# broadinstitute/permutect

Measured on AMD Instinct MI355X. Metric: read-sets/sec (train fwd+bwd), higher is better.
Workload: dtype f32 (fp32 accumulate; fwd: 2 x f16 pieces per operand = 23 bits; bwd: 2 x bf16 pieces = 16 bits)

## Files before the change

permutect_amd/csrc/pmt_phi.hip:

```cpp
#include <hip/hip_runtime.h>
#include <math.h>

#include "permutect_amd.h"

#define PHI_THREADS 256
#define PHI_MAXN (2 * PMT_MAX_ORTHO_DIM)
#define PHI_MAX_SQUARINGS 1100

__device__ double block_max(double v, double* red) {
    const int tid = threadIdx.x;
    red[tid] = v;
    __syncthreads();
    for (int s = PHI_THREADS / 2; s > 0; s >>= 1) {
        if (tid < s) red[tid] = fmax(red[tid], red[tid + s]);
        __syncthreads();
    }
    const double r = red[0];
    __syncthreads();
    return r;
}
__device__ double block_sum(double v, double* red) {
    const int tid = threadIdx.x;
    red[tid] = v;
    __syncthreads();
    for (int s = PHI_THREADS / 2; s > 0; s >>= 1) {
        if (tid < s) red[tid] += red[tid + s];
        __syncthreads();
    }
    const double r = red[0];
    __syncthreads();
    return r;
}

__device__ void matmul(double* __restrict__ Cm, const double* __restrict__ A, const double* __restrict__ B, int N, double scale) {
    for (int idx = threadIdx.x; idx < N * N; idx += PHI_THREADS) {
        const int i = idx / N, j = idx - i * N;
        double a0 = 0.0, a1 = 0.0, a2 = 0.0, a3 = 0.0;
        const double* ar = A + i * N;
        const double* bc = B + j;
        int k = 0;
        for (; k + 3 < N; k += 4) {
            a0 += ar[k] * bc[k * N];
            a1 += ar[k + 1] * bc[(k + 1) * N];
            a2 += ar[k + 2] * bc[(k + 2) * N];
            a3 += ar[k + 3] * bc[(k + 3) * N];
        }
        for (; k < N; ++k) a0 += ar[k] * bc[k * N];
        Cm[idx] = ((a0 + a1) + (a2 + a3)) * scale;
    }
    __syncthreads();
}

__device__ void expm_inplace(double* S, double* B, double* P, double* T, int N, double* red) {
    double colsum = 0.0;
    if (threadIdx.x < N)
        for (int i = 0; i < N; ++i) colsum += fabs(S[i * N + threadIdx.x]);
    const double norm1 = block_max(colsum, red);
    int s = 0;
    if (norm1 > 0.5 && norm1 <= 1.7976931348623157e308) {
        const double sq = ceil(log2(norm1 / 0.5));
        s = sq < (double)PHI_MAX_SQUARINGS ? (int)sq : PHI_MAX_SQUARINGS;
    }
    const double scale = ldexp(1.0, -s);
    for (int idx = threadIdx.x; idx < N * N; idx += PHI_THREADS) {
        const double b = S[idx] * scale;
        B[idx] = b;
        P[idx] = b;
        const int i = idx / N, j = idx - i * N;
        S[idx] = b + (i == j ? 1.0 : 0.0);
    }
    __syncthreads();
    for (int k = 2; k <= 12; ++k) {
        matmul(T, P, B, N, 1.0 / (double)k);
        for (int idx = threadIdx.x; idx < N * N; idx += PHI_THREADS) {
            P[idx] = T[idx];
            S[idx] += T[idx];
        }
        __syncthreads();
    }
    for (int q = 0; q < s; ++q) {
        matmul(T, S, S, N, 1.0);
        for (int idx = threadIdx.x; idx < N * N; idx += PHI_THREADS) S[idx] = T[idx];
        __syncthreads();
    }
}

struct PhiShared {
    double m[4][PHI_MAXN * PHI_MAXN];
    double red[PHI_THREADS];
};
static_assert(sizeof(PhiShared) <= 160 * 1024, "LDS budget");

__global__ __launch_bounds__(PHI_THREADS) void pmt_phi_forward_kernel(PmtPhiProgram prog, const float* __restrict__ theta,
                                                                       float* __restrict__ phi) {
    __shared__ __attribute__((aligned(16))) PhiShared sh;
    const PmtPhiSeg sg = prog.seg[blockIdx.x];
    const float* x = theta + sg.theta_off;
    float* y = phi + sg.phi_off;
    const int tid = threadIdx.x, n = sg.rows * sg.cols;
    if (sg.kind == PMT_PHI_EXP) {
        for (int i = tid; i < n; i += PHI_THREADS) y[i] = expf(x[i]);
    } else if (sg.kind == PMT_PHI_BOUNDED) {
        for (int i = tid; i < n; i += PHI_THREADS) y[i] = sg.p1 * (1.0f / (1.0f + expf(-x[i]))) + sg.p0;
    } else if (sg.kind == PMT_PHI_UNIT_ROWS) {
        for (int r = 0; r < sg.rows; ++r) {
            double q = 0.0;
            for (int i = tid; i < sg.cols; i += PHI_THREADS) q += (double)x[r * sg.cols + i] * (double)x[r * sg.cols + i];
            const float norm = (float)sqrt(block_sum(q, sh.red));
            for (int i = tid; i < sg.cols; i += PHI_THREADS) y[r * sg.cols + i] = x[r * sg.cols + i] / norm;
        }
    } else if (sg.kind == PMT_PHI_LOG_SOFTMAX) {
        for (int r = 0; r < sg.rows; ++r) {
            double mx = -INFINITY;
            for (int i = tid; i < sg.cols; i += PHI_THREADS) mx = fmax(mx, (double)x[r * sg.cols + i]);
            mx = block_max(mx, sh.red);
            double se = 0.0;
            for (int i = tid; i < sg.cols; i += PHI_THREADS) se += exp((double)x[r * sg.cols + i] - mx);
            const double lse = mx + log(block_sum(se, sh.red));
            for (int i = tid; i < sg.cols; i += PHI_THREADS) y[r * sg.cols + i] = (float)((double)x[r * sg.cols + i] - lse);
        }
    } else if (sg.kind == PMT_PHI_ORTHOGONAL) {
        const int N = sg.rows;
        double* S = sh.m[0];
        for (int idx = tid; idx < N * N; idx += PHI_THREADS) {
            const int i = idx / N, j = idx - i * N;
            S[idx] = i > j ? (double)x[i * N + j] : (i < j ? -(double)x[j * N + i] : 0.0);
        }
        __syncthreads();
        expm_inplace(S, sh.m[1], sh.m[2], sh.m[3], N, sh.red);
        for (int idx = tid; idx < N * N; idx += PHI_THREADS) {
            const int i = idx / N, j = idx - i * N;
            double acc = 0.0;
            if (sg.base != nullptr) {
                for (int k = 0; k < N; ++k) acc += (double)sg.base[i * sg.base_rs + k * sg.base_cs] * S[k * N + j];
            } else {
                acc = S[idx];
            }
            y[idx] = (float)acc;
        }
    }
}

__global__ __launch_bounds__(PHI_THREADS) void pmt_phi_backward_kernel(PmtPhiProgram prog, const float* __restrict__ theta,
                                                                        const float* __restrict__ phi,
                                                                        const float* __restrict__ gphi,
                                                                        float* __restrict__ gtheta) {
    __shared__ __attribute__((aligned(16))) PhiShared sh;
    const PmtPhiSeg sg = prog.seg[blockIdx.x];
    const float* x = theta + sg.theta_off;
    const float* y = phi + sg.phi_off;
    const float* gy = gphi + sg.phi_off;
    float* gx = gtheta + sg.theta_off;
    const int tid = threadIdx.x, n = sg.rows * sg.cols;
    if (sg.kind == PMT_PHI_EXP) {
        for (int i = tid; i < n; i += PHI_THREADS) gx[i] += gy[i] * y[i];
    } else if (sg.kind == PMT_PHI_BOUNDED) {
        for (int i = tid; i < n; i += PHI_THREADS) {
            const float s = 1.0f / (1.0f + expf(-x[i]));
            gx[i] += gy[i] * sg.p1 * s * (1.0f - s);
        }
    } else if (sg.kind == PMT_PHI_UNIT_ROWS) {
        for (int r = 0; r < sg.rows; ++r) {
            double q = 0.0, d = 0.0;
            for (int i = tid; i < sg.cols; i += PHI_THREADS) {
                q += (double)x[r * sg.cols + i] * (double)x[r * sg.cols + i];
                d += (double)y[r * sg.cols + i] * (double)gy[r * sg.cols + i];
            }
            const double norm = sqrt(block_sum(q, sh.red));
            const double dot = block_sum(d, sh.red);
            for (int i = tid; i < sg.cols; i += PHI_THREADS)
                gx[r * sg.cols + i] += (float)(((double)gy[r * sg.cols + i] - (double)y[r * sg.cols + i] * dot) / norm);
        }
    } else if (sg.kind == PMT_PHI_LOG_SOFTMAX) {
        for (int r = 0; r < sg.rows; ++r) {
            double g = 0.0;
            for (int i = tid; i < sg.cols; i += PHI_THREADS) g += (double)gy[r * sg.cols + i];
            const double gsum = block_sum(g, sh.red);
            for (int i = tid; i < sg.cols; i += PHI_THREADS)
                gx[r * sg.cols + i] += (float)((double)gy[r * sg.cols + i] - exp((double)y[r * sg.cols + i]) * gsum);
        }
    } else if (sg.kind == PMT_PHI_ORTHOGONAL) {
        const int nn = sg.rows, N = 2 * nn;
        double* S = sh.m[0];
        double* G = sh.m[1];
        for (int idx = tid; idx < nn * nn; idx += PHI_THREADS) {
            const int i = idx / nn, j = idx - i * nn;
            double acc = 0.0;
            if (sg.base != nullptr) {
                for (int k = 0; k < nn; ++k) acc += (double)sg.base[k * sg.base_rs + i * sg.base_cs] * (double)gy[k * nn + j];
            } else {
                acc = (double)gy[idx];
            }
            G[idx] = acc;
        }
        __syncthreads();
        for (int idx = tid; idx < N * N; idx += PHI_THREADS) {
            const int i = idx / N, j = idx - i * N;
            const int bi = i % nn, bj = j % nn;
            double v = 0.0;
            if ((i < nn) == (j < nn)) {
                v = bi > bj ? -(double)x[bi * nn + bj] : (bi < bj ? (double)x[bj * nn + bi] : 0.0);
            } else if (i < nn) {
                v = G[bi * nn + bj];
            }
            S[idx] = v;
        }
        __syncthreads();
        double* B = sh.m[1];
        expm_inplace(S, B, sh.m[2], sh.m[3], N, sh.red);
        for (int idx = tid; idx < nn * nn; idx += PHI_THREADS) {
            const int i = idx / nn, j = idx - i * nn;
            if (i > j) gx[idx] += (float)(S[i * N + nn + j] - S[j * N + nn + i]);
        }
    }
}

static int phi_check(const PmtPhiProgram* p) {
    if (!p || p->n_segs < 0 || p->n_segs > PMT_MAX_PHI_SEGS) return PMT_E_INVALID;
    for (int i = 0; i < p->n_segs; ++i) {
        const PmtPhiSeg* s = &p->seg[i];
        if (s->kind < PMT_PHI_EXP || s->kind > PMT_PHI_ORTHOGONAL || s->rows < 1 || s->cols < 1 || s->theta_off < 0 || s->phi_off < 0)
            return PMT_E_INVALID;
        if (s->kind == PMT_PHI_ORTHOGONAL && (s->rows != s->cols || s->rows > PMT_MAX_ORTHO_DIM)) return PMT_E_UNSUPPORTED;
    }
    return PMT_OK;
}

extern "C" int pmt_phi_forward(const PmtPhiProgram* prog, const float* theta, float* phi, void* stream) {
    const int rc = phi_check(prog);
    if (rc) return rc;
    if (!theta || !phi) return PMT_E_INVALID;
    if (prog->n_segs == 0) return PMT_OK;
    hipLaunchKernelGGL(pmt_phi_forward_kernel, dim3(prog->n_segs), dim3(PHI_THREADS), 0, reinterpret_cast<hipStream_t>(stream),
                       *prog, theta, phi);
    return hipGetLastError() == hipSuccess ? PMT_OK : PMT_E_LAUNCH;
}

extern "C" int pmt_phi_backward(const PmtPhiProgram* prog, const float* theta, const float* phi, const float* grad_phi,
                                float* grad_theta, void* stream) {
    const int rc = phi_check(prog);
    if (rc) return rc;
    if (!theta || !phi || !grad_phi || !grad_theta) return PMT_E_INVALID;
    if (prog->n_segs == 0) return PMT_OK;
    hipLaunchKernelGGL(pmt_phi_backward_kernel, dim3(prog->n_segs), dim3(PHI_THREADS), 0, reinterpret_cast<hipStream_t>(stream),
                       *prog, theta, phi, grad_phi, grad_theta);
    return hipGetLastError() == hipSuccess ? PMT_OK : PMT_E_LAUNCH;
}
```

Measured before the change: 20.16 million.

## Exploit block-triangular structure in orthogonal phi expm and use wave-level reductions

The backward orthogonal parametrisation no longer builds a 2n x 2n block matrix for the exponential. It tracks only the diagonal block and the upper-right Fréchet block, about a quarter of the matmul work. Small matrices that fit in one wavefront run in a single wave with wave barriers instead of block-wide syncs. Block reductions use shuffle-based wave sums with double-buffered shared slots. Ping-pong buffers remove the copy after each matmul, and a float reciprocal replaces the integer division. The gains come with more intricate indexing and a float-based row index that must stay exact for small n.

```diff
diff --git a/permutect_amd/csrc/pmt_phi.hip b/permutect_amd/csrc/pmt_phi.hip
--- a/permutect_amd/csrc/pmt_phi.hip
+++ b/permutect_amd/csrc/pmt_phi.hip
@@ -4,85 +4,163 @@
 #include "permutect_amd.h"
 
 #define PHI_THREADS 256
+#define PHI_WAVE 64
+#define PHI_WAVES (PHI_THREADS / PHI_WAVE)
 #define PHI_MAXN (2 * PMT_MAX_ORTHO_DIM)
 #define PHI_MAX_SQUARINGS 1100
-
-__device__ double block_max(double v, double* red) {
-    const int tid = threadIdx.x;
-    red[tid] = v;
+#define PHI_BLOCK_MATS 8
+
+__device__ __forceinline__ double wave_sum(double v) {
+    for (int o = PHI_WAVE / 2; o > 0; o >>= 1) v += __shfl_xor(v, o, PHI_WAVE);
+    return v;
+}
+__device__ __forceinline__ double wave_max(double v) {
+    for (int o = PHI_WAVE / 2; o > 0; o >>= 1) v = fmax(v, __shfl_xor(v, o, PHI_WAVE));
+    return v;
+}
+
+__device__ __forceinline__ double block_sum(double v, double* red, int& turn) {
+    double* r = red + PHI_WAVES * (turn++ & 1);
+    v = wave_sum(v);
+    if ((threadIdx.x & (PHI_WAVE - 1)) == 0) r[threadIdx.x / PHI_WAVE] = v;
     __syncthreads();
-    for (int s = PHI_THREADS / 2; s > 0; s >>= 1) {
-        if (tid < s) red[tid] = fmax(red[tid], red[tid + s]);
+    return (r[0] + r[1]) + (r[2] + r[3]);
+}
+__device__ __forceinline__ double block_max(double v, double* red, int& turn) {
+    double* r = red + PHI_WAVES * (turn++ & 1);
+    v = wave_max(v);
+    if ((threadIdx.x & (PHI_WAVE - 1)) == 0) r[threadIdx.x / PHI_WAVE] = v;
+    __syncthreads();
+    return fmax(fmax(r[0], r[1]), fmax(r[2], r[3]));
+}
+
+__device__ __forceinline__ void phi_sync(bool solo) {
+    if (solo) {
+        __builtin_amdgcn_fence(__ATOMIC_RELEASE, "wavefront");
+        __builtin_amdgcn_wave_barrier();
+        __builtin_amdgcn_fence(__ATOMIC_ACQUIRE, "wavefront");
+    } else {
         __syncthreads();
     }
-    const double r = red[0];
-    __syncthreads();
-    return r;
-}
-__device__ double block_sum(double v, double* red) {
-    const int tid = threadIdx.x;
-    red[tid] = v;
-    __syncthreads();
-    for (int s = PHI_THREADS / 2; s > 0; s >>= 1) {
-        if (tid < s) red[tid] += red[tid + s];
+}
+
+template <bool TWO>
+__device__ __forceinline__ double dot4(const double* __restrict__ r0, const double* __restrict__ c0, const double* __restrict__ r1,
+                                       const double* __restrict__ c1, int n) {
+    double a0 = 0.0, a1 = 0.0, a2 = 0.0, a3 = 0.0, b0 = 0.0, b1 = 0.0, b2 = 0.0, b3 = 0.0;
+    int k = 0;
+    for (; k + 3 < n; k += 4) {
+        a0 += r0[k] * c0[k * n];
+        a1 += r0[k + 1] * c0[(k + 1) * n];
+        a2 += r0[k + 2] * c0[(k + 2) * n];
+        a3 += r0[k + 3] * c0[(k + 3) * n];
+        if (TWO) {
+            b0 += r1[k] * c1[k * n];
+            b1 += r1[k + 1] * c1[(k + 1) * n];
+            b2 += r1[k + 2] * c1[(k + 2) * n];
+            b3 += r1[k + 3] * c1[(k + 3) * n];
+        }
+    }
+    if (k < n) {
+        const int k1 = k + 1 < n ? k + 1 : n - 1, k2 = k + 2 < n ? k + 2 : n - 1;
+        const double x0 = r0[k], y0 = c0[k * n], x1 = r0[k1], y1 = c0[k1 * n], x2 = r0[k2], y2 = c0[k2 * n];
+        a0 += x0 * y0;
+        a1 += k + 1 < n ? x1 * y1 : 0.0;
+        a2 += k + 2 < n ? x2 * y2 : 0.0;
+        if (TWO) {
+            const double u0 = r1[k], w0 = c1[k * n], u1 = r1[k1], w1 = c1[k1 * n], u2 = r1[k2], w2 = c1[k2 * n];
+            b0 += u0 * w0;
+            b1 += k + 1 < n ? u1 * w1 : 0.0;
+            b2 += k + 2 < n ? u2 * w2 : 0.0;
+        }
+    }
+    const double a = (a0 + a1) + (a2 + a3);
+    return TWO ? a + ((b0 + b1) + (b2 + b3)) : a;
+}
+
+template <bool WITH_F>
+__device__ __forceinline__ void block_product(double* oe, double* of, const double* le, const double* lf, const double* re, const double* rf,
+                                              double* se, double* sf, double scale, int n, int f0, int workers, float rn, bool solo) {
+    const int nn = n * n, total = WITH_F ? f0 + nn : nn;
+    for (int o = threadIdx.x; o < total; o += workers) {
+        const bool f = WITH_F && o >= f0;
+        const int idx = f ? o - f0 : o;
+        if (idx >= nn) continue;
+        const int i = (int)(((float)idx + 0.5f) * rn), j = idx - i * n;
+        if (!f) {
+            const double v = dot4<false>(le + i * n, re + j, nullptr, nullptr, n) * scale;
+            oe[idx] = v;
+            if (se) se[idx] += v;
+        } else {
+            const double v = dot4<true>(le + i * n, rf + j, lf + i * n, re + j, n) * scale;
+            of[idx] = v;
+            if (sf) sf[idx] += v;
+        }
+    }
+    phi_sync(solo);
+}
+
+template <bool WITH_F>
+__device__ double* expm_block(double* mats, int n, int workers, bool solo, double* red) {
+    const int nn = n * n, tid = threadIdx.x;
+    const float rn = 1.0f / (float)n;
+    const int f0 = solo ? nn : (nn + PHI_WAVE - 1) & ~(PHI_WAVE - 1);
+    double* Bm = mats;
+    double* Gm = mats + nn;
+    double* P[2] = {mats + 2 * nn, mats + 4 * nn};
+    double* S = mats + 6 * nn;
+    double colsum = 0.0;
+    if (tid < n) {
+        double ca = 0.0, cg = 0.0;
+        if (WITH_F)
+            for (int i = 0; i < n; ++i) cg += fabs(Gm[i * n + tid]);
+        for (int i = 0; i < n; ++i) {
+            const double a = fabs(Bm[i * n + tid]);
+            ca += a;
+            cg += a;
+        }
+        colsum = WITH_F ? fmax(ca, cg) : ca;
+    }
+    double norm1 = wave_max(colsum);
+    if (!solo) {
+        if (tid == 0) red[0] = norm1;
         __syncthreads();
-    }
-    const double r = red[0];
-    __syncthreads();
-    return r;
-}
-
-__device__ void matmul(double* __restrict__ Cm, const double* __restrict__ A, const double* __restrict__ B, int N, double scale) {
-    for (int idx = threadIdx.x; idx < N * N; idx += PHI_THREADS) {
-        const int i = idx / N, j = idx - i * N;
-        double a0 = 0.0, a1 = 0.0, a2 = 0.0, a3 = 0.0;
-        const double* ar = A + i * N;
-        const double* bc = B + j;
-        int k = 0;
-        for (; k + 3 < N; k += 4) {
-            a0 += ar[k] * bc[k * N];
-            a1 += ar[k + 1] * bc[(k + 1) * N];
-            a2 += ar[k + 2] * bc[(k + 2) * N];
-            a3 += ar[k + 3] * bc[(k + 3) * N];
-        }
-        for (; k < N; ++k) a0 += ar[k] * bc[k * N];
-        Cm[idx] = ((a0 + a1) + (a2 + a3)) * scale;
-    }
-    __syncthreads();
-}
-
-__device__ void expm_inplace(double* S, double* B, double* P, double* T, int N, double* red) {
-    double colsum = 0.0;
-    if (threadIdx.x < N)
-        for (int i = 0; i < N; ++i) colsum += fabs(S[i * N + threadIdx.x]);
-    const double norm1 = block_max(colsum, red);
+        norm1 = red[0];
+    }
     int s = 0;
     if (norm1 > 0.5 && norm1 <= 1.7976931348623157e308) {
         const double sq = ceil(log2(norm1 / 0.5));
         s = sq < (double)PHI_MAX_SQUARINGS ? (int)sq : PHI_MAX_SQUARINGS;
     }
     const double scale = ldexp(1.0, -s);
-    for (int idx = threadIdx.x; idx < N * N; idx += PHI_THREADS) {
-        const double b = S[idx] * scale;
-        B[idx] = b;
-        P[idx] = b;
-        const int i = idx / N, j = idx - i * N;
+    for (int idx = tid; idx < nn; idx += workers) {
+        const double b = Bm[idx] * scale;
+        const int i = (int)(((float)idx + 0.5f) * rn), j = idx - i * n;
+        Bm[idx] = b;
+        P[0][idx] = b;
         S[idx] = b + (i == j ? 1.0 : 0.0);
-    }
-    __syncthreads();
+        if (WITH_F) {
+            const double g = Gm[idx] * scale;
+            Gm[idx] = g;
+            P[0][nn + idx] = g;
+            S[nn + idx] = g;
+        }
+    }
+    phi_sync(solo);
+    int cur = 0;
     for (int k = 2; k <= 12; ++k) {
-        matmul(T, P, B, N, 1.0 / (double)k);
-        for (int idx = threadIdx.x; idx < N * N; idx += PHI_THREADS) {
-            P[idx] = T[idx];
-            S[idx] += T[idx];
-        }
-        __syncthreads();
-    }
+        block_product<WITH_F>(P[cur ^ 1], P[cur ^ 1] + nn, P[cur], P[cur] + nn, Bm, Gm, S, S + nn, 1.0 / (double)k, n, f0, workers, rn, solo);
+        cur ^= 1;
+    }
+    double* R = S;
+    double* T = P[0];
     for (int q = 0; q < s; ++q) {
-        matmul(T, S, S, N, 1.0);
-        for (int idx = threadIdx.x; idx < N * N; idx += PHI_THREADS) S[idx] = T[idx];
-        __syncthreads();
-    }
+        block_product<WITH_F>(T, T + nn, R, R + nn, R, R + nn, nullptr, nullptr, 1.0, n, f0, workers, rn, solo);
+        double* t = R;
+        R = T;
+        T = t;
+    }
+    return R;
 }
 
 struct PhiShared {
@@ -90,6 +168,11 @@
     double red[PHI_THREADS];
 };
 static_assert(sizeof(PhiShared) <= 160 * 1024, "LDS budget");
+static_assert(PHI_BLOCK_MATS * PMT_MAX_ORTHO_DIM * PMT_MAX_ORTHO_DIM <= 4 * PHI_MAXN * PHI_MAXN, "expm_block's work matrices fit PhiShared::m");
+static_assert(PMT_MAX_ORTHO_DIM <= PHI_WAVE, "expm_block reduces the column sums in wave 0");
+static_assert(PHI_WAVES == 4 && 2 * PHI_WAVES <= PHI_THREADS, "block_sum / block_max add four waves' values from two halves of `red`");
+
+__device__ __forceinline__ bool phi_solo(int outputs) { return outputs <= PHI_WAVE; }
 
 __global__ __launch_bounds__(PHI_THREADS) void pmt_phi_forward_kernel(PmtPhiProgram prog, const float* __restrict__ theta,
                                                                        float* __restrict__ phi) {
@@ -98,6 +181,7 @@
     const float* x = theta + sg.theta_off;
     float* y = phi + sg.phi_off;
     const int tid = threadIdx.x, n = sg.rows * sg.cols;
+    int turn = 0;
     if (sg.kind == PMT_PHI_EXP) {
         for (int i = tid; i < n; i += PHI_THREADS) y[i] = expf(x[i]);
     } else if (sg.kind == PMT_PHI_BOUNDED) {
@@ -106,35 +190,39 @@
         for (int r = 0; r < sg.rows; ++r) {
             double q = 0.0;
             for (int i = tid; i < sg.cols; i += PHI_THREADS) q += (double)x[r * sg.cols + i] * (double)x[r * sg.cols + i];
-            const float norm = (float)sqrt(block_sum(q, sh.red));
+            const float norm = (float)sqrt(block_sum(q, sh.red, turn));
             for (int i = tid; i < sg.cols; i += PHI_THREADS) y[r * sg.cols + i] = x[r * sg.cols + i] / norm;
         }
     } else if (sg.kind == PMT_PHI_LOG_SOFTMAX) {
         for (int r = 0; r < sg.rows; ++r) {
             double mx = -INFINITY;
             for (int i = tid; i < sg.cols; i += PHI_THREADS) mx = fmax(mx, (double)x[r * sg.cols + i]);
-            mx = block_max(mx, sh.red);
+            mx = block_max(mx, sh.red, turn);
             double se = 0.0;
             for (int i = tid; i < sg.cols; i += PHI_THREADS) se += exp((double)x[r * sg.cols + i] - mx);
-            const double lse = mx + log(block_sum(se, sh.red));
+            const double lse = mx + log(block_sum(se, sh.red, turn));
             for (int i = tid; i < sg.cols; i += PHI_THREADS) y[r * sg.cols + i] = (float)((double)x[r * sg.cols + i] - lse);
         }
     } else if (sg.kind == PMT_PHI_ORTHOGONAL) {
         const int N = sg.rows;
-        double* S = sh.m[0];
-        for (int idx = tid; idx < N * N; idx += PHI_THREADS) {
-            const int i = idx / N, j = idx - i * N;
-            S[idx] = i > j ? (double)x[i * N + j] : (i < j ? -(double)x[j * N + i] : 0.0);
-        }
-        __syncthreads();
-        expm_inplace(S, sh.m[1], sh.m[2], sh.m[3], N, sh.red);
-        for (int idx = tid; idx < N * N; idx += PHI_THREADS) {
-            const int i = idx / N, j = idx - i * N;
+        const bool solo = phi_solo(N * N);
+        if (solo && tid >= PHI_WAVE) return;
+        const int workers = solo ? PHI_WAVE : PHI_THREADS;
+        const float rn = 1.0f / (float)N;
+        double* mats = &sh.m[0][0];
+        for (int idx = tid; idx < N * N; idx += workers) {
+            const int i = (int)(((float)idx + 0.5f) * rn), j = idx - i * N;
+            mats[idx] = i > j ? (double)x[i * N + j] : (i < j ? -(double)x[j * N + i] : 0.0);
+        }
+        phi_sync(solo);
+        const double* Q = expm_block<false>(mats, N, workers, solo, sh.red);
+        for (int idx = tid; idx < N * N; idx += workers) {
+            const int i = (int)(((float)idx + 0.5f) * rn), j = idx - i * N;
             double acc = 0.0;
             if (sg.base != nullptr) {
-                for (int k = 0; k < N; ++k) acc += (double)sg.base[i * sg.base_rs + k * sg.base_cs] * S[k * N + j];
+                for (int k = 0; k < N; ++k) acc += (double)sg.base[i * sg.base_rs + k * sg.base_cs] * Q[k * N + j];
             } else {
-                acc = S[idx];
+                acc = Q[idx];
             }
             y[idx] = (float)acc;
         }
@@ -152,6 +240,7 @@
     const float* gy = gphi + sg.phi_off;
     float* gx = gtheta + sg.theta_off;
     const int tid = threadIdx.x, n = sg.rows * sg.cols;
+    int turn = 0;
     if (sg.kind == PMT_PHI_EXP) {
         for (int i = tid; i < n; i += PHI_THREADS) gx[i] += gy[i] * y[i];
     } else if (sg.kind == PMT_PHI_BOUNDED) {
@@ -166,8 +255,8 @@
                 q += (double)x[r * sg.cols + i] * (double)x[r * sg.cols + i];
                 d += (double)y[r * sg.cols + i] * (double)gy[r * sg.cols + i];
             }
-            const double norm = sqrt(block_sum(q, sh.red));
-            const double dot = block_sum(d, sh.red);
+            const double norm = sqrt(block_sum(q, sh.red, turn));
+            const double dot = block_sum(d, sh.red, turn);
             for (int i = tid; i < sg.cols; i += PHI_THREADS)
                 gx[r * sg.cols + i] += (float)(((double)gy[r * sg.cols + i] - (double)y[r * sg.cols + i] * dot) / norm);
         }
@@ -175,16 +264,21 @@
         for (int r = 0; r < sg.rows; ++r) {
             double g = 0.0;
             for (int i = tid; i < sg.cols; i += PHI_THREADS) g += (double)gy[r * sg.cols + i];
-            const double gsum = block_sum(g, sh.red);
+            const double gsum = block_sum(g, sh.red, turn);
             for (int i = tid; i < sg.cols; i += PHI_THREADS)
                 gx[r * sg.cols + i] += (float)((double)gy[r * sg.cols + i] - exp((double)y[r * sg.cols + i]) * gsum);
         }
     } else if (sg.kind == PMT_PHI_ORTHOGONAL) {
-        const int nn = sg.rows, N = 2 * nn;
-        double* S = sh.m[0];
-        double* G = sh.m[1];
-        for (int idx = tid; idx < nn * nn; idx += PHI_THREADS) {
-            const int i = idx / nn, j = idx - i * nn;
+        const int nn = sg.rows;
+        const bool solo = phi_solo(2 * nn * nn);
+        if (solo && tid >= PHI_WAVE) return;
+        const int workers = solo ? PHI_WAVE : PHI_THREADS;
+        const float rn = 1.0f / (float)nn;
+        double* mats = &sh.m[0][0];
+        double* G = mats + nn * nn;
+        for (int idx = tid; idx < nn * nn; idx += workers) {
+            const int i = (int)(((float)idx + 0.5f) * rn), j = idx - i * nn;
+            mats[idx] = i > j ? -(double)x[i * nn + j] : (i < j ? (double)x[j * nn + i] : 0.0);
             double acc = 0.0;
             if (sg.base != nullptr) {
                 for (int k = 0; k < nn; ++k) acc += (double)sg.base[k * sg.base_rs + i * sg.base_cs] * (double)gy[k * nn + j];
@@ -193,24 +287,11 @@
             }
             G[idx] = acc;
         }
-        __syncthreads();
-        for (int idx = tid; idx < N * N; idx += PHI_THREADS) {
-            const int i = idx / N, j = idx - i * N;
-            const int bi = i % nn, bj = j % nn;
-            double v = 0.0;
-            if ((i < nn) == (j < nn)) {
-                v = bi > bj ? -(double)x[bi * nn + bj] : (bi < bj ? (double)x[bj * nn + bi] : 0.0);
-            } else if (i < nn) {
-                v = G[bi * nn + bj];
-            }
-            S[idx] = v;
-        }
-        __syncthreads();
-        double* B = sh.m[1];
-        expm_inplace(S, B, sh.m[2], sh.m[3], N, sh.red);
-        for (int idx = tid; idx < nn * nn; idx += PHI_THREADS) {
-            const int i = idx / nn, j = idx - i * nn;
-            if (i > j) gx[idx] += (float)(S[i * N + nn + j] - S[j * N + nn + i]);
+        phi_sync(solo);
+        const double* F = expm_block<true>(mats, nn, workers, solo, sh.red) + nn * nn;
+        for (int idx = tid; idx < nn * nn; idx += workers) {
+            const int i = (int)(((float)idx + 0.5f) * rn), j = idx - i * nn;
+            if (i > j) gx[idx] += (float)(F[i * nn + j] - F[j * nn + i]);
         }
     }
 }
```

Measured after the change: 20.31 million, median of 6. No clear change (+0.8%).
